# JacobYoung115/VisualSLAM

Hardware: AMD Instinct MI355X
Metric: frames/sec @1080p (Harris + DoG keypoint detection) (higher is better)
Workload: dtype u8

## Files before the change

### visualslam_amd/csrc/kernels_aux.hip.h

```cpp
#pragma once
#include <hip/hip_runtime.h>

#include "kernels_generic.hip.h"
#include "kernels_localize.hip.h"

namespace vslam {

__global__ __launch_bounds__(256) void k_resize_linear2x_slide(const uint8_t* __restrict__ src, size_t sstep, size_t sframe,
                                                                uint8_t* __restrict__ dst, size_t dframe, int dpitch,
                                                                int rows, int cols, int seg) {
    const int k = blockIdx.x * 256 + threadIdx.x;
    if (4 * k >= cols) return;
    const bool whole = 4 * k + 3 < cols;
    const int m0 = blockIdx.y * seg, m1 = min(m0 + seg, rows);
    const uint8_t* s = src + blockIdx.z * sframe;
    uint8_t* d = dst + blockIdx.z * dframe + 8 * k;
    const int xl = max(4 * k - 1, 0), xr = min(4 * k + 4, cols - 1);
    auto hrow = [&](int m, uint32_t (&X)[4], uint32_t (&Y)[4]) {
        const uint8_t* r = s + (size_t)min(max(m, 0), rows - 1) * sstep;
        uint32_t w;
        if (whole)
            __builtin_memcpy(&w, r + 4 * k, 4);
        else
            w = (uint32_t)r[4 * k] | ((uint32_t)r[min(4 * k + 1, cols - 1)] << 8) | ((uint32_t)r[min(4 * k + 2, cols - 1)] << 16) |
                ((uint32_t)r[cols - 1] << 24);
        const uint32_t s0 = r[xl], s5 = r[xr];
        const uint32_t P = __builtin_amdgcn_perm(w, w, 0x0c010c00);
        const uint32_t Q = __builtin_amdgcn_perm(w, w, 0x0c030c02);
        const uint32_t Qm = __builtin_amdgcn_perm(w, w, 0x0c020c01);
        const uint32_t Pm = s0 | ((w & 0xffu) << 16);
        const uint32_t Qp = (w >> 24) | (s5 << 16);
        const uint32_t P3 = P + (P << 1), Q3 = Q + (Q << 1);
        const uint32_t A[4] = {Pm + P3, P3 + Qm, Qm + Q3, Q3 + Qp};
#pragma unroll
        for (int i = 0; i < 4; ++i) {
            X[i] = pk_lshr_u16(A[i], 2);
            Y[i] = pk_lshr_u16(A[i] + (A[i] << 1), 2);
        }
    };
    auto emit = [&](int dy, const uint32_t (&U)[4], const uint32_t (&V)[4]) {
        uint32_t v[4];
#pragma unroll
        for (int i = 0; i < 4; ++i) v[i] = pk_lshr_u16(U[i] + V[i] + 0x00020002u, 2);
        *reinterpret_cast<uint2*>(d + (size_t)dy * dpitch) = make_uint2(v[0] | (v[1] << 8), v[2] | (v[3] << 8));
    };
    uint32_t Xp[4], Yp[4], Xc[4], Yc[4];
    hrow(m0 - 1, Xp, Yp);
    hrow(m0, Xc, Yc);
    for (int m = m0; m < m1; ++m) {
        uint32_t Xn[4], Yn[4];
        hrow(m + 1, Xn, Yn);
        emit(2 * m, Xp, Yc);
        emit(2 * m + 1, Yc, Xn);
#pragma unroll
        for (int i = 0; i < 4; ++i) Xp[i] = Xc[i], Xc[i] = Xn[i], Yc[i] = Yn[i];
    }
}

__global__ __launch_bounds__(256) void k_resize_nearest_half_v4(const uint8_t* __restrict__ src, size_t sframe, int spitch,
                                                                 uint8_t* __restrict__ dst, size_t dframe, int dpitch,
                                                                 int rows, int drows, int dcols) {
    const int k = blockIdx.x * 256 + threadIdx.x;
    const int y = blockIdx.y;
    if (4 * k >= dcols) return;
    const int sy = min(2 * y, rows - 1);
    const uint2 w = *reinterpret_cast<const uint2*>(src + blockIdx.z * sframe + (size_t)sy * spitch + 8 * k);
    *reinterpret_cast<uint32_t*>(dst + blockIdx.z * dframe + (size_t)y * dpitch + 4 * k) =
        even_bytes(w.x, w.y);
}

constexpr int EXT_SPAN = 768;
constexpr int EXT_PITCH = EXT_SPAN + 16;

template <bool LOC>
__global__ __launch_bounds__(256) void k_extrema_w3(const uint8_t* __restrict__ pyr, size_t pframe, ExtGeom g, int o,
                                                     unsigned long long* __restrict__ bits,
                                                     unsigned long long* __restrict__ lflags, size_t bframe, int li0, int li_step) {
    constexpr int NROW = LOC ? 13 : 10;
    __shared__ __attribute__((aligned(16))) uint8_t srow[NROW * EXT_PITCH + 16];
    __shared__ uint2 queue[LOC ? 768 : 1];
    __shared__ uint8_t qkeep[LOC ? 768 : 1];
    const int li = li0 + (int)blockIdx.y * li_step, f = blockIdx.z;
    const int rows = g.rows[o], cols = g.cols[o], pitch = g.pitch[o];
    const uint32_t P = (uint32_t)rows * (uint32_t)pitch;
    const uint8_t* dog = pyr + f * pframe + g.oct_off[o] + (size_t)VSLAM_NUM_LEVELS * P;
    const int ya = max(3 * li - 1, 0), yb = 3 * li;
    const int yc = min(3 * li + 1, rows - 1);
    const int c0 = blockIdx.x * EXT_SPAN - 16;
    const int wave = __builtin_amdgcn_readfirstlane(threadIdx.x >> 6), lane = threadIdx.x & 63;
    const int cpiece = c0 + 16 * lane;
    const bool piece_ok = lane < EXT_PITCH / 16 && cpiece >= 0 && cpiece < cols;
#pragma unroll
    for (int i = 0; i < (NROW + 3) / 4; ++i) {
        const int rl = wave + 4 * i;
        if (rl < NROW) {
            const int lev = rl < 10 ? (rl >> 1) : rl - 9, y = rl < 10 ? ((rl & 1) ? yb : ya) : yc;
            const uint8_t* rowp = dog + (ptrdiff_t)(int)((uint32_t)lev * P + (uint32_t)y * (uint32_t)pitch + (uint32_t)c0);
            if (piece_ok)
                *reinterpret_cast<uint4*>(srow + rl * EXT_PITCH + 16 * lane) =
                    *reinterpret_cast<const uint4*>(rowp + (uint32_t)(16 * lane));
        }
    }
    if (blockIdx.x == 0 && threadIdx.x < 10)
        srow[threadIdx.x * EXT_PITCH + 15] = dog[(threadIdx.x >> 1) * P + (uint32_t)((threadIdx.x & 1) ? yb : ya) * (uint32_t)pitch];
    __syncthreads();
    const int lc = g.lat_cols[o], wpr = g.wpr[o], lr = g.lat_rows[o];
    const int lj = blockIdx.x * 256 + threadIdx.x;
    bool cand[3] = {false, false, false}, listed[3] = {false, false, false};
    unsigned long long wcand[3], wlist[3];
    const unsigned long long owns = __builtin_amdgcn_ballot_w64(lj < lc);
    const int xa = 3 * (int)threadIdx.x - 1 + 16;
    uint32_t self[5];
    uint32_t up[5], left[5];
    {
        const uint32_t s = xa & 3;
        const uint32_t sel = 0x0c000c00u | s | ((s + 1) << 16);
        uint32_t mn[5], mx[5];
#pragma unroll
        for (int l = 0; l < 5; ++l) {
            uint32_t off = (uint32_t)(xa & ~3) + (uint32_t)(2 * l * EXT_PITCH);
            if (l) asm volatile("" : "+v"(off));
            const uint32_t* q0 = reinterpret_cast<const uint32_t*>(srow + off);
            const uint32_t* q1 = q0 + EXT_PITCH / 4;
            const uint32_t v0 = __builtin_amdgcn_perm(q0[1], q0[0], sel), v1 = __builtin_amdgcn_perm(q1[1], q1[0], sel);
            const uint32_t lo = pk_min_u16(v0, v1), hi = pk_max_u16(v0, v1);
            mn[l] = min(lo & 0xffffu, lo >> 16);
            mx[l] = max(hi & 0xffffu, hi >> 16);
            self[l] = v1 >> 16;
            if (LOC) up[l] = v0 >> 16, left[l] = v1 & 0xffffu;
        }
#pragma unroll
        for (int L = 1; L <= 3; ++L) {
            const uint32_t lo = min(mn[L - 1], min(mn[L], mn[L + 1])), hi = max(mx[L - 1], max(mx[L], mx[L + 1]));
            wcand[L - 1] = (__builtin_amdgcn_ballot_w64(self[L] == lo) | __builtin_amdgcn_ballot_w64(self[L] == hi)) & owns;
            if (LOC) cand[L - 1] = lj < lc && (self[L] == lo || self[L] == hi);
            else wlist[L - 1] = wcand[L - 1] & __builtin_amdgcn_ballot_w64((int)self[L] >= g.min_contrast);
        }
    }
    if (LOC) {
        uint2* wq = queue + wave * 192;
        uint8_t* wk = qkeep + wave * 192;
        const int xj = xa + 1;
        const int xr = xj + ((3 * lj + 1 < cols) ? 1 : 0);
        unsigned int nw = 0;
        bool queued[3];
#pragma unroll
        for (int L = 1; L <= 3; ++L) {
            bool nz = false;
            uint32_t dpack = 0;
            if (cand[L - 1]) {
                const uint8_t* r1 = srow + (2 * L + 1) * EXT_PITCH;
                const uint8_t* r2 = srow + (9 + L) * EXT_PITCH;
                const int d_x = (int)left[L] - (int)r1[xr];
                const int d_y = (int)up[L] - (int)r2[xj];
                const int d_s = (int)self[L - 1] - (int)self[L + 1];
                nz = d_x != 0 && d_y != 0 && d_s != 0;
                listed[L - 1] = !nz && self[L] >= 8u;
                dpack = (uint32_t)(d_x + 256) | ((uint32_t)(d_y + 256) << 10) | ((uint32_t)(d_s + 256) << 20);
            }
            const unsigned long long m = __builtin_amdgcn_ballot_w64(nz);
            if (nz) {
                const unsigned int slot = nw + __builtin_amdgcn_mbcnt_hi((uint32_t)(m >> 32), __builtin_amdgcn_mbcnt_lo((uint32_t)m, 0u));
                wq[slot] = make_uint2(dpack, self[L] | ((uint32_t)((L - 1) * 64 + lane) << 8));
            }
            queued[L - 1] = nz;
            nw += (unsigned int)__builtin_popcountll(m);
        }
        if (nw) {
            __builtin_amdgcn_fence(__ATOMIC_RELEASE, "wavefront");
            __builtin_amdgcn_wave_barrier();
            __builtin_amdgcn_fence(__ATOMIC_ACQUIRE, "wavefront");
            for (unsigned int q = lane; q < nw; q += 64) {
                const uint2 e = wq[q];
                int nv;
                wk[e.y >> 8] = feature_point_localization((int)(e.x & 1023u) - 256, (int)((e.x >> 10) & 1023u) - 256,
                                                          (int)(e.x >> 20) - 256, (int)(e.y & 255u), nv, g.loc_lut);
            }
            __builtin_amdgcn_fence(__ATOMIC_RELEASE, "wavefront");
            __builtin_amdgcn_wave_barrier();
            __builtin_amdgcn_fence(__ATOMIC_ACQUIRE, "wavefront");
#pragma unroll
            for (int L = 0; L < 3; ++L)
                if (queued[L]) listed[L] = wk[L * 64 + lane] != 0;
        }
    }
    const int word = blockIdx.x * 4 + wave;
    if (word < wpr) {
        const size_t w0 = f * bframe + g.bits_off[o] + (size_t)li * wpr + word;
#pragma unroll
        for (int L = 0; L < 3; ++L) {
            const unsigned long long wc = wcand[L], wl = LOC ? __builtin_amdgcn_ballot_w64(listed[L]) : wlist[L];
            if (lane == 0) {
                const size_t w = w0 + (size_t)L * lr * wpr;
                if (bits) bits[w] = wc;
                lflags[w] = wl;
            }
        }
    }
}


template <bool FMA>
__device__ __forceinline__ float mad_f32(float a, float b, float c) {
    if constexpr (FMA) return __builtin_fmaf(a, b, c);
    else return a * b + c;
}

template <bool FMA = false>
__device__ __forceinline__ float fast_atan2_deg(float y, float x) {
    const float scale = (float)(180.0 / 3.14159265358979323846);
    const float p1 = 0.9997878412794807f * scale, p3 = -0.3258083974640975f * scale;
    const float p5 = 0.1555786518463281f * scale, p7 = -0.04432655554792128f * scale;
    const float eps = (float)2.2204460492503131e-16;
    const float ax = fabsf(x), ay = fabsf(y);
    float a;
    if (ax >= ay) {
        const float c = ay / (ax + eps), c2 = c * c;
        a = mad_f32<FMA>(mad_f32<FMA>(mad_f32<FMA>(p7, c2, p5), c2, p3), c2, p1) * c;
    } else {
        const float c = ax / (ay + eps), c2 = c * c;
        a = 90.f - mad_f32<FMA>(mad_f32<FMA>(mad_f32<FMA>(p7, c2, p5), c2, p3), c2, p1) * c;
    }
    if (x < 0) a = 180.f - a;
    if (y < 0) a = 360.f - a;
    return a;
}

template <bool FMA>
__global__ __launch_bounds__(256) void k_level_gradients(const uint8_t* __restrict__ g, int gpitch, int rows, int cols,
                                                          float* __restrict__ gx, float* __restrict__ gy,
                                                          float* __restrict__ mag, float* __restrict__ orient) {
    const int c = blockIdx.x * 256 + threadIdx.x;
    const int r = blockIdx.y;
    if (c >= cols) return;
    float x, y;
    gradient_at(g, gpitch, rows, cols, r, c, x, y);
    const size_t o = (size_t)r * cols + c;
    if (gx) gx[o] = x;
    if (gy) gy[o] = y;
    if (mag) {
        const float xx = x * x, yy = y * y;
        mag[o] = sqrt_rn_small_nr(xx + yy);
    }
    if (orient) orient[o] = fast_atan2_deg<FMA>(y, x);
}

}
```

### visualslam_amd/csrc/vslam_hip.hip

```cpp
#include <hip/hip_runtime.h>

#include <algorithm>
#include <cstdio>
#include <cstdlib>
#include <cstring>
#include <deque>
#include <functional>
#include <map>
#include <string>
#include <set>
#include <memory>
#include <vector>

#include "../../include/vslam.h"
#include "kernels_generic.hip.h"
#include "kernels_pyramid.hip.h"
#include "kernels_strip.hip.h"
#include "kernels_hdiff.hip.h"
#include "kernels_aux.hip.h"
#include "kernels_harris_strip.hip.h"
#include "kernels_orient.hip.h"
#include "kernels_orient_batch.hip.h"
#include "kernels_orient_pk.hip.h"
#include "kernels_compact.hip.h"
#include "kernels_sift.hip.h"
#include "kernels_extrema_dense.hip.h"
#include "vslam_internal.h"
#include "vslam_ctx.h"
#include "vslam_launch.h"
#include "vslam_mx.h"
#include "vslam_octave_launch.h"

using namespace vslam;


struct vslam_pyramid {
    vslam_ctx* ctx = nullptr;
    vslam_params params{};
    vslam_batch_layout layout{};
    vslam_pyramid_info info{};
    uint8_t* d_block = nullptr;
    uint8_t* d_bases = nullptr;
    size_t block_cap = 0, bases_cap = 0;
    size_t base_off[VSLAM_MAX_OCTAVES] = {};
};


static const char* const kKernelNames =
    "k_resize_linear2x\nk_blur_h_generic\nk_blur_v_generic\n"
    "k_dog5\nk_resize_nearest_half\nk_extrema\nk_pyr_octave\nk_pyr_octave_mx\n"
    "k_gauss_v_strip\nk_gauss_h_strip\nk_gauss_h_diff\nk_resize_linear2x_slide\nk_resize_nearest_half_v4\nk_extrema_w3\nk_extrema_dense\nk_localize_points\nk_orient_keypoints\nk_edge_response_windows\nk_level_gradients\nk_pack_rows\nk_edge_flags\nk_survivor_ranges\nk_orient_survivors\n"
    "k_extrema_pack\nk_harris_strip\nk_flag_count\nk_chunk_scan\nk_flag_scatter\nk_level_gradients\nk_sift_descriptors\nk_pack_offsets\nk_pack_copy\nk_count_totals\n"
    "k_desc_norms\nk_match_nn2\nk_match_merge";


struct StreamSwap {
    vslam_ctx* c;
    hipStream_t saved;
    StreamSwap(vslam_ctx* ctx, hipStream_t s) : c(ctx), saved(ctx->stream) { c->stream = s; }
    ~StreamSwap() { c->stream = saved; }
};

static int raise_dyn_lds(vslam_ctx* c, const void* fn) {
    if (c->lds_raised.count(fn)) return VSLAM_OK;
    HIPCHK(c, hipFuncSetAttribute(fn, hipFuncAttributeMaxDynamicSharedMemorySize, kMaxDynLds));
    c->lds_raised.insert(fn);
    return VSLAM_OK;
}

static void* block_alloc(vslam_ctx* c, size_t bytes, size_t* cap) {
    int best = -1;
    for (int i = 0; i < (int)c->block_cache.size(); ++i) {
        const size_t sz = c->block_cache[i].first;
        if (sz >= bytes && sz <= 2 * bytes + (1 << 20) && (best < 0 || sz < c->block_cache[best].first)) best = i;
    }
    if (best >= 0) {
        void* p = c->block_cache[best].second;
        *cap = c->block_cache[best].first;
        c->block_cache.erase(c->block_cache.begin() + best);
        return p;
    }
    void* p = nullptr;
    if (hipMalloc(&p, bytes) != hipSuccess) {
        for (auto& b : c->block_cache) (void)hipFree(b.second);
        c->block_cache.clear();
        if (hipMalloc(&p, bytes) != hipSuccess) return nullptr;
    }
    *cap = bytes;
    return p;
}
static void block_release(vslam_ctx* c, void* p, size_t cap) {
    if (!p) return;
    if (c && c->block_cache.size() < 8 && cap <= ((size_t)1 << 30))
        c->block_cache.emplace_back(cap, p);
    else
        (void)hipFree(p);
}

int vslam::ws_reserve(vslam_ctx* c, size_t bytes) {
    if (bytes <= c->ws_cap) return VSLAM_OK;
    HIPCHK(c, hipStreamSynchronize(c->stream));
    for (int i = 0; i < vslam_ctx::kAux; ++i)
        if (c->aux[i]) HIPCHK(c, hipStreamSynchronize(c->aux[i]));
    if (c->ws) (void)hipFree(c->ws);
    c->ws = nullptr;
    c->ws_cap = 0;
    const size_t want = align_up(bytes + bytes / 8, 1 << 20);
    HIPCHK(c, hipMalloc((void**)&c->ws, want));
    c->ws_cap = want;
    return VSLAM_OK;
}

static bool stream_is_capturing(vslam_ctx* c) {
    hipStreamCaptureStatus cap = hipStreamCaptureStatusNone;
    if (hipStreamIsCapturing(c->stream, &cap) != hipSuccess) (void)hipGetLastError();
    return cap != hipStreamCaptureStatusNone;
}
#define NO_TABLE_IN_CAPTURE(ctx, what)                                                                                                      \
    if (stream_is_capturing(ctx))                                                                                                           \
    return fail(ctx, VSLAM_ERR_UNSUPPORTED, std::string(what) + ": its tap tables are not on the device yet and cannot be put there during a stream capture - " \
                                                                "run one warm-up call with the same parameters and the same matrix-path setting first")

enum TableKind { kTableBlur, kTableStrip, kTableTile, kTableMx, kTableOrient };

template <class T, class Fill>
static int get_table(vslam_ctx* c, TableKind kind, double v, int i, const char* what, size_t bytes, Fill fill, const T** out) {
    uint64_t vb;
    std::memcpy(&vb, &v, 8);
    const auto key = std::make_tuple((int)kind, vb, i);
    auto it = c->tables.find(key);
    if (it == c->tables.end()) {
        NO_TABLE_IN_CAPTURE(c, what);
        std::vector<char> host(bytes);
        TRY(fill(static_cast<void*>(host.data())));
// ... 262 lines not shown
    ws.add(s.bases, (size_t)nf * sum_p);
    ws.add(s.h, (size_t)nf * dog_h_elems(L, plans) + 128);
    ws.add(s.lflags, (size_t)nf * L.bits_frame_words);
    ws.add(s.cws, compaction_ws_elems(L.bits_frame_words, nf));
    ws.add(s.pbegin, nf);
}


template <class CFG>
static int enqueue_pyr_octave(vslam_ctx* c, double sigma0, int o, const OctPlan& pl, const OctIO& io) {
    const PyrTaps<CFG>* taps;
    TRY(get_table(c, kTableTile, sigma0, o, "octave kernel", sizeof(PyrTaps<CFG>), [&](void* host) -> int {
        const uint16_t* tp[6];
        tap_pointers(pl.taps, tp);
        pyr_pack_taps<CFG>(tp, *static_cast<PyrTaps<CFG>*>(host));
        return VSLAM_OK;
    }, &taps));
    TRY(raise_dyn_lds(c, reinterpret_cast<const void*>(&k_pyr_octave<CFG>)));
    const dim3 grid((io.cols + CFG::TW - 1) / CFG::TW, (io.rows + CFG::TH - 1) / CFG::TH, io.nf);
    LAUNCH_ON(c, "k_pyr_octave", o, c->stream, CFG::LDS_BYTES, k_pyr_octave<CFG>, grid, dim3(CFG::NT), io.base, io.bframe, io.oct, io.pframe, io.rows,
              io.cols, io.pitch, taps, io.next_base, io.nframe, io.nrows, io.ncols, io.npitch);
    return VSLAM_OK;
}

static int enqueue_pyr_octave_mx(vslam_ctx* c, double sigma0, int o, const OctPlan& pl, const OctIO& io, const MxScan* scan, int up2_step = 0) {
    const void* table;
    TRY(get_table(c, kTableMx, sigma0, o, "matrix-core octave kernel", mx_taps_bytes(pl.mx), [&](void* host) -> int {
        const uint16_t* tp[6];
        tap_pointers(pl.taps, tp);
        if (!mx_pack(pl.mx, tp, host)) return fail(c, VSLAM_ERR_UNSUPPORTED, "matrix-core octave kernel: a tap exceeds 127");
        HIPCHK(c, mx_prepare(pl.mx));
        return VSLAM_OK;
    }, &table));
    hipError_t e;
    {
        TimedScope ts(c, "k_pyr_octave_mx", o);
        e = mx_launch(pl.mx, c->stream, table, io, scan, up2_step);
    }
    HIPCHK(c, e);
    return VSLAM_OK;
}

static int dog_side_gate(const std::vector<OctPlan>& plans, int nf) {
    int gate = -1;
    if (nf >= 32)
        for (int o = 0; o < (int)plans.size(); ++o)
            if (plans[o].path == OctPath::Tile0 || plans[o].path == OctPath::Tile1) gate = o;
    return gate;
}

static DenseGeom dense_geom(const vslam_batch_layout& L, int o, int min_contrast, int nf) {
    DenseGeom g;
    g.rows = L.rows[o], g.cols = L.cols[o], g.pitch = L.pitch[o];
    g.wpr = (g.cols + 63) / 64;
    g.min_contrast = min_contrast;
    g.P = (unsigned int)((size_t)g.rows * g.pitch);
    g.dog_off = (unsigned int)(L.octave_offset[o] + (size_t)VSLAM_NUM_LEVELS * g.P);
    const long waves_per_rowseg = 4L * (((g.cols + 3) / 4 + 255) / 256) * nf;
    const long segs_wanted = std::max<long>(1, 8192 / waves_per_rowseg);
    g.seg = (int)std::min<long>(XD_SEG_MAX, std::max<long>(4, (g.rows + segs_wanted - 1) / segs_wanted));
    return g;
}

namespace {
struct DogOut {
    uint8_t* pyr;
    size_t pframe;
    unsigned long long* bits = nullptr;
    bool do_extrema = false;
    vslam_point* points = nullptr;
    unsigned int* counts = nullptr;
};

struct DogRun {
    hipStream_t side = nullptr;
    hipStream_t up = nullptr;
    std::function<int(int)> after_list;
    std::function<int(int)> after_octave;
    bool later_chunk = false;
    bool bases_are_scratch = false;
};
}

static int enqueue_octave_scan(vslam_ctx* c, const vslam_params& p, const vslam_batch_layout& L, const ExtGeom& g, const DogScratch& s,
                               const MxScan* fused, int o, int o_done, int nf, const DogOut& out, const DogRun& run) {
    uint8_t* const pyr = out.pyr;
    const size_t pframe = out.pframe;
    unsigned long long* const bits = out.bits;
    const hipStream_t side = run.side;
    if (out.do_extrema && L.lat_rows[o] > 0 && L.lat_cols[o] > 0) {
        hipStream_t es = c->stream;
        if (side) {
            HIPCHK(c, hipStreamWaitEvent(side, c->ev_oct[o_done], 0));
            es = side;
        }
        if (p.extrema_dense) {
            const DenseGeom dg = dense_geom(L, o, p.min_contrast, nf);
            hipLaunchKernelGGL(k_extrema_dense, dim3(((dg.cols + 3) / 4 + 255) / 256, (dg.rows + dg.seg - 1) / dg.seg, nf), dim3(256), 0, es,
                               pyr, pframe, dg, bits ? bits + L.bits_offset[o] : nullptr, s.lflags + L.bits_offset[o], L.bits_frame_words);
        } else if (fused) {
            {
                TimedScope ts(c, "k_extrema_pack", o, es);
                HIPCHK(c, mx_launch_pack(es, *fused, L.rows[o], L.lat_words[o], nf, bits ? bits + L.bits_offset[o] : nullptr, s.lflags + L.bits_offset[o],
                                         L.bits_frame_words, kMxStripRows));
            }
            const int sr = kMxStripRows;
            const int n_straddle = (L.lat_rows[o] - 1) / sr;
            TimedScope ts(c, "k_extrema_w3", o, es);
            if (n_straddle > 0)
                hipLaunchKernelGGL(k_extrema_w3<false>, dim3((L.lat_words[o] + 3) / 4, n_straddle, nf), dim3(256), 0, es, pyr, pframe, g, o, bits, s.lflags,
                                   L.bits_frame_words, sr, sr);
            if (es != c->stream) {
                HIPCHK(c, hipEventRecord(c->ev_pack, es));
                c->pack_pending = true;
            }
        } else if (p.extrema_window == 3) {
            const dim3 eg((L.lat_words[o] + 3) / 4, L.lat_rows[o], nf);
            if (p.localize)
                LAUNCH_ON(c, "k_extrema_w3", o, es, 0, k_extrema_w3<true>, eg, dim3(256), pyr, pframe, g, o, bits, s.lflags, L.bits_frame_words, 0, 1);
            else
                LAUNCH_ON(c, "k_extrema_w3", o, es, 0, k_extrema_w3<false>, eg, dim3(256), pyr, pframe, g, o, bits, s.lflags, L.bits_frame_words, 0, 1);
        } else
            hipLaunchKernelGGL(k_extrema, dim3((L.lat_cols[o] + 255) / 256, L.lat_rows[o], nf * 3), dim3(256), 0, es, pyr,
                               pframe, g, o, bits, s.lflags, L.bits_frame_words);
        HIPCHK(c, hipGetLastError());
    }
    if (out.do_extrema && out.points && out.counts) {
        StreamSwap sw(c, side ? side : c->stream);
        const size_t entries = (size_t)3 * L.lat_rows[o] * L.lat_words[o];
        if (p.extrema_dense) {
            DenseDogEntries ent{s.lflags + L.bits_offset[o], L.bits_frame_words, pyr, pframe, dense_geom(L, o, p.min_contrast, nf), o, out.points};
            TRY(enqueue_compaction(c, ent, entries, nf, s.cws, p.dog_cap, out.counts, o > 0 ? 1 : 0));
        } else {
            DogEntries ent{s.lflags, L.bits_frame_words, pyr, pframe, g, o, o + 1, out.points};
            TRY(enqueue_compaction(c, ent, entries, nf, s.cws, p.dog_cap, out.counts, o > 0 ? 1 : 0));
        }
        if (run.after_list) TRY(run.after_list(o));
    }
    return VSLAM_OK;
}

static int enqueue_dog(vslam_ctx* c, const vslam_params& p, const vslam_batch_layout& L, const std::vector<OctPlan>& plans, const uint8_t* frames,
                       size_t fstep, size_t fframe, int nf, DogScratch& s, const DogOut& out, const DogRun& run = DogRun()) {
    const hipStream_t side = run.side, up = run.up;
    const int gate = (side && p.localize) ? dog_side_gate(plans, nf) : -1;
    ExtGeom g;
    if (p.localize) TRY(ensure_loc_lut(c));
    fill_geom(c, p, L, g);
    const bool up2_fused = c->mx && run.bases_are_scratch && L.n_octaves > 0 && L.rows[0] == 2 * p.rows && L.cols[0] == 2 * p.cols && fstep <= 0x7fffffff &&
                           mx_up2_supported(plans[0].mx);
    const int nf_a = (!up2_fused && side && up && nf >= 64) ? nf / 2 : nf;
    if (!up2_fused)
        LAUNCH(c, "k_resize_linear2x_slide", k_resize_linear2x_slide, dim3(((p.cols + 3) / 4 + 255) / 256, (p.rows + 15) / 16, nf_a), dim3(256),
               frames, fstep, fframe, s.bases + s.base_off[0], s.bases_frame, L.pitch[0], p.rows, p.cols, 16);
    if (nf_a < nf) {
        if (run.later_chunk) HIPCHK(c, hipStreamWaitEvent(up, c->ev_chunk, 0));
        StreamSwap sw(c, up);
        LAUNCH(c, "k_resize_linear2x_slide", k_resize_linear2x_slide, dim3(((p.cols + 3) / 4 + 255) / 256, (p.rows + 15) / 16, nf - nf_a), dim3(256),
               frames + (size_t)nf_a * fframe, fstep, fframe, s.bases + s.base_off[0] + (size_t)nf_a * s.bases_frame, s.bases_frame, L.pitch[0],
               p.rows, p.cols, 16);
        HIPCHK(c, hipEventRecord(c->ev_up2, c->stream));
    }
    bool fused[VSLAM_MAX_OCTAVES] = {};
    if (run.later_chunk && c->pack_pending) {
        HIPCHK(c, hipStreamWaitEvent(c->stream, c->ev_pack, 0));
        c->pack_pending = false;
    }
    MxScan scan[VSLAM_MAX_OCTAVES] = {};
    struct TagReset {
        vslam_ctx* c;
        ~TagReset() { c->launch_tag = -1; }
    } tag_reset{c};
    for (int o = 0; o < L.n_octaves; ++o) {
        c->launch_tag = o;
        const int rows = L.rows[o], cols = L.cols[o], pitch = L.pitch[o];
        const size_t P = (size_t)rows * pitch;
        const OctPlan& pl = plans[o];
        const bool has_next = o + 1 < L.n_octaves;
        const bool fuse_next = has_next && pl.path != OctPath::Generic;
        OctIO io{s.bases + s.base_off[o], s.bases_frame, out.pyr + L.octave_offset[o], out.pframe, rows, cols, pitch, nf,
                 fuse_next ? s.bases + s.base_off[o + 1] : nullptr, s.bases_frame, has_next ? L.rows[o + 1] : 0, has_next ? L.cols[o + 1] : 0,
                 has_next ? L.pitch[o + 1] : 0};
        if (o == 0 && up2_fused) io.base = frames, io.bframe = fframe;
        const int shape = pyr_tile_wide(rows, cols) ? 1 : 0;
        fused[o] = c->mx && s.sitemap && out.do_extrema && !p.localize && !p.extrema_dense && p.extrema_window == 3 && L.lat_rows[o] > 0 &&
                   L.lat_cols[o] > 0 && mx_scan_supported(pl.mx);
        if (fused[o])
            scan[o] = MxScan{s.sitemap + s.site_off[o], s.site_frame, L.lat_rows[o], L.lat_cols[o], s.site_pitch[o], p.min_contrast,
                             s.colmap + s.col_off[o], s.col_frame, mx_seams(cols)};
        auto tiled = [&](int f_lo, int n) -> int {
            const OctIO part = io.frames(f_lo, n);
            if (c->mx && pl.mx) {
                MxScan sc = scan[o];
                if (fused[o]) sc.sitemap += (size_t)f_lo * s.site_frame, sc.colmap += (size_t)f_lo * s.col_frame;
                return enqueue_pyr_octave_mx(c, p.sigma0, o, pl, part, fused[o] ? &sc : nullptr, o == 0 && up2_fused ? (int)fstep : 0);
            }
            if (pl.path == OctPath::Tile0)
                return shape == 1 ? enqueue_pyr_octave<PyrCfgOct0W>(c, p.sigma0, o, pl, part) : enqueue_pyr_octave<PyrCfgOct0>(c, p.sigma0, o, pl, part);
            return shape == 1 ? enqueue_pyr_octave<PyrCfgOct1W>(c, p.sigma0, o, pl, part) : enqueue_pyr_octave<PyrCfgOct1>(c, p.sigma0, o, pl, part);
        };
        const bool is_tiled = pl.path == OctPath::Tile0 || pl.path == OctPath::Tile1 || (c->mx && pl.mx != 0);
        if (o == 0 && nf_a < nf && !is_tiled) HIPCHK(c, hipStreamWaitEvent(c->stream, c->ev_up2, 0));
        if (is_tiled && o == 0 && nf_a < nf) {
            TRY(tiled(0, nf_a));
// ... 461 lines not shown
    TRY(d2h(c, dst, dst_step, d_src, cols, cols, rows));
    return vslam_ctx_sync(c);
}

int vslam_pyramid_get_base(const vslam_pyramid* py, int octave, uint8_t* dst, size_t dst_step) {
    if (!py) return VSLAM_ERR_INVALID;
    if (octave < 0 || octave >= py->layout.n_octaves) return fail(py->ctx, VSLAM_ERR_RANGE, "octave out of range");
    return pyramid_fetch(py, octave, py->d_bases + py->base_off[octave], dst, dst_step);
}

int vslam_pyramid_get_gauss(const vslam_pyramid* py, int octave, int level, uint8_t* dst, size_t dst_step) {
    if (!py) return VSLAM_ERR_INVALID;
    if (octave < 0 || octave >= py->layout.n_octaves || level < 0 || level >= VSLAM_NUM_LEVELS)
        return fail(py->ctx, VSLAM_ERR_RANGE, "octave/level out of range");
    const size_t P = (size_t)py->layout.rows[octave] * py->layout.pitch[octave];
    return pyramid_fetch(py, octave, py->d_block + py->layout.octave_offset[octave] + (size_t)level * P, dst, dst_step);
}

int vslam_pyramid_get_dog(const vslam_pyramid* py, int octave, int level, uint8_t* dst, size_t dst_step) {
    if (!py) return VSLAM_ERR_INVALID;
    if (octave < 0 || octave >= py->layout.n_octaves || level < 0 || level >= VSLAM_NUM_DOGS)
        return fail(py->ctx, VSLAM_ERR_RANGE, "octave/level out of range");
    const size_t P = (size_t)py->layout.rows[octave] * py->layout.pitch[octave];
    return pyramid_fetch(py, octave,
                         py->d_block + py->layout.octave_offset[octave] + (size_t)(VSLAM_NUM_LEVELS + level) * P, dst,
                         dst_step);
}

int vslam_pyramid_get_gradients(const vslam_pyramid* py, int octave, int level, float* grad_x, float* grad_y, float* mag,
                                float* orient, size_t dst_step) {
    if (!py) return VSLAM_ERR_INVALID;
    vslam_ctx* c = py->ctx;
    TRY(bind_device(c));
    if (octave < 0 || octave >= py->layout.n_octaves || level < 0 || level >= VSLAM_NUM_LEVELS)
        return fail(c, VSLAM_ERR_RANGE, "octave/level out of range");
    const int rows = py->layout.rows[octave], cols = py->layout.cols[octave];
    ARGCHK(c, dst_step >= 4 * (size_t)cols, "pyramid gradients: bad destination step");
    float* host[4] = {grad_x, grad_y, mag, orient};
    const size_t P = (size_t)rows * cols;
    float* dev[4];
    WsPlan ws;
    for (int i = 0; i < 4; ++i) ws.add(dev[i], P);
    TRY(ws.commit(c));
    for (int i = 0; i < 4; ++i)
        if (!host[i]) dev[i] = nullptr;
    const int pitch = py->layout.pitch[octave];
    const uint8_t* g = py->d_block + py->layout.octave_offset[octave] + (size_t)level * rows * pitch;
    if (c->f32_fused)
        LAUNCH(c, "k_level_gradients", k_level_gradients<true>, grid_rows(cols, rows), dim3(256), g, pitch, rows, cols, dev[0], dev[1], dev[2], dev[3]);
    else
        LAUNCH(c, "k_level_gradients", k_level_gradients<false>, grid_rows(cols, rows), dim3(256), g, pitch, rows, cols, dev[0], dev[1], dev[2], dev[3]);
    for (int i = 0; i < 4; ++i)
        if (host[i]) TRY(d2h(c, host[i], dst_step, dev[i], 4 * (size_t)cols, 4 * (size_t)cols, rows));
    return vslam_ctx_sync(c);
}

static int dog_points_host(vslam_ctx* c, const vslam_pyramid* py, int octave, int window, int min_contrast, int localize,
                           uint64_t* bits, vslam_point* out, size_t cap, size_t* count) {
    TRY(bind_device(c));
    ARGCHK(c, py && py->ctx == c && count && (out || cap == 0), "initialKeypointDetection: bad arguments");
    if (octave < 0 || octave >= py->layout.n_octaves) return fail(c, VSLAM_ERR_RANGE, "octave out of range");
    ARGCHK(c, window >= 3 && (window & 1), "initialKeypointDetection: windowSize must be odd and >= 3");
    vslam_params p = py->params;
    p.extrema_window = window;
    p.min_contrast = min_contrast;
    p.localize = localize;
    p.dog_cap = (uint32_t)std::min<size_t>(cap, 0x7fffffff);
    vslam_batch_layout L;
    if (make_layout(&p, &L) != VSLAM_OK) return fail(c, VSLAM_ERR_INVALID, "bad extrema parameters");
    ExtGeom g;
    if (p.localize) TRY(ensure_loc_lut(c));
    fill_geom(c, p, L, g);
    const size_t words = L.bits_frame_words;
    unsigned long long *d_bits, *d_lf;
    vslam_point* d_pts;
    unsigned int *d_n, *d_cws;
    WsPlan ws;
    ws.add(d_bits, words), ws.add(d_lf, words), ws.add(d_pts, p.dog_cap), ws.add(d_n, 1), ws.add(d_cws, compaction_ws_elems(words, 1));
    TRY(ws.commit(c));
    HIPCHK(c, hipMemsetAsync(d_n, 0, 4, c->stream));
    const size_t ow = (size_t)3 * L.lat_rows[octave] * L.lat_words[octave];
    if (ow) {
        if (window == 3) {
            const dim3 eg((L.lat_words[octave] + 3) / 4, L.lat_rows[octave], 1);
            if (localize)
                LAUNCH(c, "k_extrema_w3", k_extrema_w3<true>, eg, dim3(256), py->d_block, L.pyramid_frame_bytes, g, octave, d_bits, d_lf, words, 0, 1);
            else
                LAUNCH(c, "k_extrema_w3", k_extrema_w3<false>, eg, dim3(256), py->d_block, L.pyramid_frame_bytes, g, octave, d_bits, d_lf, words, 0, 1);
        } else {
            LAUNCH(c, "k_extrema", k_extrema, dim3((L.lat_cols[octave] + 255) / 256, L.lat_rows[octave], 3), dim3(256),
                   py->d_block, L.pyramid_frame_bytes, g, octave, d_bits, d_lf, words);
        }
        DogEntries ent{d_lf, words, py->d_block, L.pyramid_frame_bytes, g, octave, octave + 1, d_pts};
        TRY(enqueue_compaction(c, ent, ow, 1, d_cws, p.dog_cap, d_n, 0));
    }
    return read_list(c, d_n, d_pts, p.dog_cap, out, count, bits, d_bits + L.bits_offset[octave], bits ? ow * 8 : 0);
}

int vslam_dog_extrema(vslam_ctx* c, const vslam_pyramid* py, int octave, int window, int min_contrast, uint64_t* bits,
                      vslam_point* out, size_t cap, size_t* count) {
    return dog_points_host(c, py, octave, window, min_contrast, 0, bits, out, cap, count);
}

int vslam_dog_extrema_dense(vslam_ctx* c, const vslam_pyramid* py, int octave, int min_contrast, uint64_t* bits,
                            vslam_point* out, size_t cap, size_t* count) {
    TRY(bind_device(c));
    ARGCHK(c, py && py->ctx == c && count && (out || cap == 0), "dense extrema: bad arguments");
    if (octave < 0 || octave >= py->layout.n_octaves) return fail(c, VSLAM_ERR_RANGE, "octave out of range");
    ARGCHK(c, min_contrast >= 0 && min_contrast <= 65535, "dense extrema: min_contrast out of range");
    const vslam_batch_layout& L = py->layout;
    DenseGeom g = dense_geom(L, octave, min_contrast, 1);
    const size_t words = (size_t)3 * g.rows * g.wpr;
    const unsigned int ocap = (unsigned int)std::min<size_t>(cap, 0x7fffffff);
    unsigned long long *d_bits, *d_lf;
    vslam_point* d_pts;
    unsigned int *d_n, *d_cws;
    WsPlan ws;
    ws.add(d_bits, words), ws.add(d_lf, words), ws.add(d_pts, ocap), ws.add(d_n, 1), ws.add(d_cws, compaction_ws_elems(words, 1));
    TRY(ws.commit(c));
    HIPCHK(c, hipMemsetAsync(d_n, 0, 4, c->stream));
    LAUNCH(c, "k_extrema_dense", k_extrema_dense, dim3(((g.cols + 3) / 4 + 255) / 256, (g.rows + g.seg - 1) / g.seg, 1), dim3(256),
           py->d_block, L.pyramid_frame_bytes, g, bits ? d_bits : nullptr, d_lf, words);
    DenseDogEntries ent{d_lf, words, py->d_block, L.pyramid_frame_bytes, g, octave, d_pts};
    TRY(enqueue_compaction(c, ent, words, 1, d_cws, ocap, d_n, 0));
    return read_list(c, d_n, d_pts, ocap, out, count, bits, d_bits, bits ? words * 8 : 0);
}

int vslam_dog_keypoints(vslam_ctx* c, const vslam_pyramid* py, int octave, int window, vslam_point* out, size_t cap,
                        size_t* count) {
    return dog_points_host(c, py, octave, window, 0, 1, nullptr, out, cap, count);
}

int vslam_localize_points(vslam_ctx* c, const int* diffs, size_t n, int* keep, int* value) {
    TRY(bind_device(c));
    ARGCHK(c, (diffs && keep && value) || n == 0, "FeaturePointLocalization: bad arguments");
    ARGCHK(c, n <= 0x7fffffff, "FeaturePointLocalization: too many points");
    if (n == 0) return VSLAM_OK;
    int4* d_in;
    int2* d_out;
    WsPlan ws;
    ws.add(d_in, n), ws.add(d_out, n);
    TRY(ws.commit(c));
    HIPCHK(c, hipMemcpyAsync(d_in, diffs, 16 * n, hipMemcpyHostToDevice, c->stream));
    TRY(ensure_loc_lut(c));
    LAUNCH(c, "k_localize_points", k_localize_points, dim3((unsigned)((n + 255) / 256)), dim3(256), d_in, (int)n, d_out, c->loc_lut);
    std::vector<int2> h(n);
    HIPCHK(c, hipMemcpyAsync(h.data(), d_out, 8 * n, hipMemcpyDeviceToHost, c->stream));
    TRY(vslam_ctx_sync(c));
    for (size_t i = 0; i < n; ++i) keep[i] = h[i].x, value[i] = h[i].y;
    return VSLAM_OK;
}

int vslam_filter_keypoints(vslam_ctx* c, const vslam_pyramid* py, int octave, const vslam_point* kps, size_t n,
                           vslam_point* out, size_t cap, size_t* count) {
    TRY(bind_device(c));
    ARGCHK(c, py && py->ctx == c && count && (kps || n == 0) && (out || cap == 0), "filterKeypoints: bad arguments");
    if (octave < 0 || octave >= py->layout.n_octaves) return fail(c, VSLAM_ERR_RANGE, "octave out of range");
    ARGCHK(c, n <= 0x7fffffff, "filterKeypoints: too many keypoints");
    *count = 0;
    if (n == 0) return VSLAM_OK;
    const int rows = py->layout.rows[octave], cols = py->layout.cols[octave], pitch = py->layout.pitch[octave];
    const size_t P = (size_t)rows * cols;
    bool used[VSLAM_NUM_LEVELS] = {};
    for (size_t i = 0; i < n; ++i) {
        const vslam_point& k = kps[i];
        if (k.level < 0 || k.level >= VSLAM_NUM_LEVELS || k.col < 0 || k.row < 0 || k.col > cols || k.row > rows || k.octave != octave)
            return fail(c, VSLAM_ERR_RANGE, "filterKeypoints: keypoint outside the octave's data");
        used[k.level] = true;
    }
    std::vector<float> taps[VSLAM_NUM_LEVELS];
    int max_r = 0;
// ... 577 lines not shown
```

### visualslam_amd/csrc/vslam_octave_launch.h

```cpp
#pragma once
#include <algorithm>
#include <cstddef>
#include <initializer_list>

namespace vslam {

constexpr int STRIP_W = 64;
constexpr int HD_J = 16;
constexpr int HD_PAD = 2;
constexpr int kMaxDynLds = 150 * 1024;

struct StripVGeom {
    int RM, rhq;
    size_t lds;
};
constexpr StripVGeom strip_v_geom(int rows, int nmax) {
    const int RM = (nmax / 2 + 3) & ~3;
    const int rhq = (((rows + 3) & ~3) + 2 * RM + 16) / 4;
    return StripVGeom{RM, rhq, (size_t)rhq * STRIP_W * 4};
}

constexpr int strip_pw(int cols, int nmax) { return ((cols + 7) / 2 + nmax / 2 + 12 + 3) & ~3; }

constexpr int strip_item_capacity(int RI) { return RI == 4 ? 512 : 1024; }

constexpr int strip_sh(int cols) { return cols <= 1024 ? 16 : cols <= 2048 ? 8 : cols <= 4096 ? 4 : 0; }

constexpr int strip_plan_sh(int rows, int cols, int nmax) {
    const int sh = strip_sh(cols);
    return sh && strip_v_geom(rows, nmax).lds <= (size_t)kMaxDynLds && (size_t)sh * strip_pw(cols, nmax) * 4 <= (size_t)kMaxDynLds ? sh : 0;
}

constexpr int hd_left_halo(int rmax) { return (rmax + 2 + 15) & ~15; }
constexpr int hd_pw(int cols, int HL, int rmax) {
    const int ccount = HL + 16 * ((cols + HD_J - 1) / HD_J) + rmax;
    return (ccount + 1 + 15) / 16 * (16 + HD_PAD);
}
constexpr bool hdiff_fits(int cols) { return (cols + HD_J - 1) / HD_J <= 256; }

struct StripLaunch {
    int lsplit;
    size_t v_lds;
    bool diff;
    int npairs;
    int SH, RI;
    int h_grid_y;
    size_t h_lds;
    int pw;
};

inline StripLaunch strip_launch(int rows, int cols, int nf, int sh, bool hdiff, int nmax, int hd_HL = 0, int hd_rmax = 0) {
    StripLaunch s{};
    s.v_lds = strip_v_geom(rows, nmax).lds;
    const int strips = (cols + STRIP_W - 1) / STRIP_W;
    const int want = (256 + strips * nf - 1) / (strips * nf);
    s.lsplit = want >= 6 ? 6 : want >= 3 ? 3 : want >= 2 ? 2 : 1;
    if (hdiff) {
        const int ncs = (cols + HD_J - 1) / HD_J;
        s.pw = hd_pw(cols, hd_HL, hd_rmax);
        int npairs = std::max(1, std::min(8, 256 / ncs));
        while (npairs > 1 && ((size_t)npairs * s.pw * 8 > (size_t)kMaxDynLds || (long)((rows + 2 * npairs - 1) / (2 * npairs)) * nf < 256)) --npairs;
        s.diff = true;
        s.npairs = npairs;
        s.h_grid_y = (rows + 2 * npairs - 1) / (2 * npairs);
        s.h_lds = (size_t)npairs * s.pw * 8;
        return s;
    }
    s.pw = strip_pw(cols, nmax);
    while (sh > 4 && (long)((rows + sh - 1) / sh) * nf < 256) sh >>= 1;
    int ri = 4;
    if (sh == 4 && (long)((rows + 3) / 4) * nf < 256 && ((cols + 7) / 8) * 4 <= 512) {
        ri = 1;
    } else if (sh == 16) {
        const int ncg = (cols + 7) / 8;
        auto waste = [&](int r) {
            const long items = (long)ncg * (16 / r);
            if (items > strip_item_capacity(r)) return 1e9;
            return (double)((items + 63) / 64 * 64 - items) / (double)items;
        };
        for (int r : {2, 1})
            if (waste(r) + 0.02 < waste(ri)) ri = r;
    }
    s.SH = sh;
    s.RI = ri;
    s.h_grid_y = (rows + sh - 1) / sh;
    s.h_lds = (size_t)sh * s.pw * 4;
    return s;
}

constexpr bool pyr_tile_wide(int rows, int cols) {
    return (long)((cols + 255) / 256) * ((rows + 31) / 32) <= (long)((cols + 127) / 128) * ((rows + 63) / 64);
}

}
```

Baseline: 14580.

## Add paired-row 3x3x3 extrema scan kernel processing two lattice rows per block

Adds k_extrema_w3_pairs, a 128-thread kernel that stages four DoG rows per level into LDS and evaluates two lattice rows per block. It uses byte-perm packing and packed 16-bit min/max to test both rows at once, sharing the overlapping middle rows. A launch helper picks this path for full, non-localized scans and otherwise falls back to the existing kernel. The aim is fewer redundant row loads and less per-row launch overhead, at the cost of smaller blocks and extra bookkeeping for the edge guard and odd row counts.

```diff
diff --git a/visualslam_amd/csrc/kernels_aux.hip.h b/visualslam_amd/csrc/kernels_aux.hip.h
--- a/visualslam_amd/csrc/kernels_aux.hip.h
+++ b/visualslam_amd/csrc/kernels_aux.hip.h
@@ -3,6 +3,7 @@
 
 #include "kernels_generic.hip.h"
 #include "kernels_localize.hip.h"
+#include "vslam_octave_launch.h"
 
 namespace vslam {
 
@@ -69,8 +70,6 @@
         even_bytes(w.x, w.y);
 }
 
-constexpr int EXT_SPAN = 768;
-constexpr int EXT_PITCH = EXT_SPAN + 16;
 
 template <bool LOC>
 __global__ __launch_bounds__(256) void k_extrema_w3(const uint8_t* __restrict__ pyr, size_t pframe, ExtGeom g, int o,
@@ -199,6 +198,90 @@
     }
 }
 
+typedef __attribute__((address_space(3))) uint32_t lds_u32;
+struct __attribute__((aligned(8))) ExtPiece {
+    uint2 lo, hi;
+};
+
+__global__ __launch_bounds__(EXT2_SITES) void k_extrema_w3_pairs(const uint8_t* __restrict__ pyr, size_t pframe, ExtGeom g, int o,
+                                                                  unsigned long long* __restrict__ bits,
+                                                                  unsigned long long* __restrict__ lflags, size_t bframe) {
+    __shared__ __attribute__((aligned(16))) uint8_t srow[EXT2_ROWS * EXT2_PITCH];
+    const int li = 2 * (int)blockIdx.y, f = blockIdx.z;
+    const int rows = g.rows[o], cols = g.cols[o], pitch = g.pitch[o];
+    const uint32_t P = (uint32_t)rows * (uint32_t)pitch;
+    const int wave = __builtin_amdgcn_readfirstlane(threadIdx.x >> 6), lane = threadIdx.x & 63;
+    const int c0 = (int)blockIdx.x * EXT2_SPAN - EXT2_GUARD;
+    {
+        const int y0 = wave ? min(3 * li + 2, rows - 1) : max(3 * li - 1, 0), y1 = wave ? min(3 * li + 3, rows - 1) : 3 * li;
+        const uint8_t* lev = pyr + f * pframe + g.oct_off[o] + (size_t)VSLAM_NUM_LEVELS * P + (ptrdiff_t)c0;
+        const uint32_t o0 = (uint32_t)y0 * (uint32_t)pitch, o1 = (uint32_t)y1 * (uint32_t)pitch;
+        const int at = min(min(16 * lane, EXT2_PITCH - 16), pitch - 16 - c0);
+        const bool piece_ok = 16 * lane < EXT2_PITCH && c0 + 16 * lane < cols;
+        uint8_t* dst = srow + (2 * wave) * EXT2_PITCH + at;
+#pragma unroll
+        for (int l = 0; l < 5; ++l) {
+            if (piece_ok) {
+                ExtPiece a = *reinterpret_cast<const ExtPiece*>(lev + o0 + (uint32_t)at);
+                ExtPiece b = *reinterpret_cast<const ExtPiece*>(lev + o1 + (uint32_t)at);
+                *reinterpret_cast<ExtPiece*>(dst + (4 * l) * EXT2_PITCH) = a;
+                *reinterpret_cast<ExtPiece*>(dst + (4 * l + 1) * EXT2_PITCH) = b;
+            }
+            lev += P;
+        }
+    }
+    __syncthreads();
+    if (blockIdx.x == 0) {
+        if (threadIdx.x < EXT2_ROWS) srow[threadIdx.x * EXT2_PITCH + EXT2_GUARD - 1] = srow[threadIdx.x * EXT2_PITCH + EXT2_GUARD];
+        __syncthreads();
+    }
+    const int lc = g.lat_cols[o], wpr = g.wpr[o], lr = g.lat_rows[o];
+    const int lj = (int)blockIdx.x * EXT2_SITES + (int)threadIdx.x;
+    const unsigned long long owns = __builtin_amdgcn_ballot_w64(lj < lc);
+    const uint32_t xa = 3u * threadIdx.x + (EXT2_GUARD - 1), xb = xa + 1;
+    const uint32_t sela = 0x0c040c00u + (xa & 3) * 0x00010001u, selb = 0x0c040c00u + (xb & 3) * 0x00010001u;
+    const uint8_t* pa = srow + (xa & ~3u);
+    const uint8_t* pb = srow + (xb & ~3u);
+    uint32_t mn[5], mx[5], self[5];
+#pragma unroll
+    for (int l = 0; l < 5; ++l) {
+        uint32_t a[4], b[4];
+#pragma unroll
+        for (int r = 0; r < 4; ++r) {
+            a[r] = *(const volatile lds_u32*)(pa + (4 * l + r) * EXT2_PITCH);
+            b[r] = *(const volatile lds_u32*)(pb + (4 * l + r) * EXT2_PITCH);
+        }
+        const uint32_t a02 = __builtin_amdgcn_perm(a[2], a[0], sela), b02 = __builtin_amdgcn_perm(b[2], b[0], selb);
+        const uint32_t a13 = __builtin_amdgcn_perm(a[3], a[1], sela), b13 = __builtin_amdgcn_perm(b[3], b[1], selb);
+        mn[l] = pk_min_u16(pk_min_u16(a02, b02), pk_min_u16(a13, b13));
+        mx[l] = pk_max_u16(pk_max_u16(a02, b02), pk_max_u16(a13, b13));
+        self[l] = b13;
+    }
+    unsigned long long wc[3][2], wl[3][2];
+#pragma unroll
+    for (int L = 1; L <= 3; ++L) {
+        const uint32_t lo = pk_min_u16(mn[L - 1], pk_min_u16(mn[L], mn[L + 1])), hi = pk_max_u16(mx[L - 1], pk_max_u16(mx[L], mx[L + 1]));
+        const uint32_t s0 = self[L] & 0xffffu, s1 = self[L] >> 16;
+        wc[L - 1][0] = (__builtin_amdgcn_ballot_w64(s0 == (lo & 0xffffu)) | __builtin_amdgcn_ballot_w64(s0 == (hi & 0xffffu))) & owns;
+        wc[L - 1][1] = (__builtin_amdgcn_ballot_w64(s1 == (lo >> 16)) | __builtin_amdgcn_ballot_w64(s1 == (hi >> 16))) & owns;
+        wl[L - 1][0] = wc[L - 1][0] & __builtin_amdgcn_ballot_w64((int)s0 >= g.min_contrast);
+        wl[L - 1][1] = wc[L - 1][1] & __builtin_amdgcn_ballot_w64((int)s1 >= g.min_contrast);
+    }
+    const int word = (int)blockIdx.x * 2 + wave;
+    if (word < wpr && lane == 0) {
+        const int nrow = li + 1 < lr ? 2 : 1;
+        const size_t w0 = f * bframe + g.bits_off[o] + (size_t)((uint32_t)li * (uint32_t)wpr + (uint32_t)word);
+        const size_t lstep = (uint32_t)lr * (uint32_t)wpr;
+        for (int r = 0; r < nrow; ++r) {
+            unsigned long long* lf = lflags + w0 + (uint32_t)(r * wpr);
+            lf[0] = r ? wl[0][1] : wl[0][0], lf[lstep] = r ? wl[1][1] : wl[1][0], lf[2 * lstep] = r ? wl[2][1] : wl[2][0];
+            if (bits) {
+                unsigned long long* bt = bits + w0 + (uint32_t)(r * wpr);
+                bt[0] = r ? wc[0][1] : wc[0][0], bt[lstep] = r ? wc[1][1] : wc[1][0], bt[2 * lstep] = r ? wc[2][1] : wc[2][0];
+            }
+        }
+    }
+}
 
 template <bool FMA>
 __device__ __forceinline__ float mad_f32(float a, float b, float c) {
diff --git a/visualslam_amd/csrc/vslam_hip.hip b/visualslam_amd/csrc/vslam_hip.hip
--- a/visualslam_amd/csrc/vslam_hip.hip
+++ b/visualslam_amd/csrc/vslam_hip.hip
@@ -49,7 +49,7 @@
 static const char* const kKernelNames =
     "k_resize_linear2x\nk_blur_h_generic\nk_blur_v_generic\n"
     "k_dog5\nk_resize_nearest_half\nk_extrema\nk_pyr_octave\nk_pyr_octave_mx\n"
-    "k_gauss_v_strip\nk_gauss_h_strip\nk_gauss_h_diff\nk_resize_linear2x_slide\nk_resize_nearest_half_v4\nk_extrema_w3\nk_extrema_dense\nk_localize_points\nk_orient_keypoints\nk_edge_response_windows\nk_level_gradients\nk_pack_rows\nk_edge_flags\nk_survivor_ranges\nk_orient_survivors\n"
+    "k_gauss_v_strip\nk_gauss_h_strip\nk_gauss_h_diff\nk_resize_linear2x_slide\nk_resize_nearest_half_v4\nk_extrema_w3\nk_extrema_w3_pairs\nk_extrema_dense\nk_localize_points\nk_orient_keypoints\nk_edge_response_windows\nk_level_gradients\nk_pack_rows\nk_edge_flags\nk_survivor_ranges\nk_orient_survivors\n"
     "k_extrema_pack\nk_harris_strip\nk_flag_count\nk_chunk_scan\nk_flag_scatter\nk_level_gradients\nk_sift_descriptors\nk_pack_offsets\nk_pack_copy\nk_count_totals\n"
     "k_desc_norms\nk_match_nn2\nk_match_merge";
 
@@ -478,6 +478,26 @@
 };
 }
 
+#ifdef VSLAM_DIAGNOSTICS
+static bool g_scan_pairs = true;
+extern "C" __attribute__((visibility("default"))) void vslam_diag_scan_pairs(int on) { g_scan_pairs = on != 0; }
+#else
+static constexpr bool g_scan_pairs = true;
+#endif
+
+static int launch_scan_w3(vslam_ctx* c, hipStream_t st, const uint8_t* pyr, size_t pframe, const ExtGeom& g, int o, bool localize, int li0, int li_step,
+                          int n_rows, int nf, unsigned long long* bits, unsigned long long* lflags, size_t bframe) {
+    const ScanLaunch sl = scan_launch(g.lat_rows[o], g.lat_cols[o], localize, li0, li_step, n_rows, g_scan_pairs);
+    const dim3 grid(sl.grid_x, sl.grid_y, nf), block(sl.threads);
+    if (sl.pairs)
+        LAUNCH_ON(c, "k_extrema_w3", o, st, 0, k_extrema_w3_pairs, grid, block, pyr, pframe, g, o, bits, lflags, bframe);
+    else if (localize)
+        LAUNCH_ON(c, "k_extrema_w3", o, st, 0, k_extrema_w3<true>, grid, block, pyr, pframe, g, o, bits, lflags, bframe, li0, li_step);
+    else
+        LAUNCH_ON(c, "k_extrema_w3", o, st, 0, k_extrema_w3<false>, grid, block, pyr, pframe, g, o, bits, lflags, bframe, li0, li_step);
+    return VSLAM_OK;
+}
+
 static int enqueue_octave_scan(vslam_ctx* c, const vslam_params& p, const vslam_batch_layout& L, const ExtGeom& g, const DogScratch& s,
                                const MxScan* fused, int o, int o_done, int nf, const DogOut& out, const DogRun& run) {
     uint8_t* const pyr = out.pyr;
@@ -502,20 +522,16 @@
             }
             const int sr = kMxStripRows;
             const int n_straddle = (L.lat_rows[o] - 1) / sr;
-            TimedScope ts(c, "k_extrema_w3", o, es);
             if (n_straddle > 0)
-                hipLaunchKernelGGL(k_extrema_w3<false>, dim3((L.lat_words[o] + 3) / 4, n_straddle, nf), dim3(256), 0, es, pyr, pframe, g, o, bits, s.lflags,
-                                   L.bits_frame_words, sr, sr);
+                TRY(launch_scan_w3(c, es, pyr, pframe, g, o, false, sr, sr, n_straddle, nf, bits, s.lflags, L.bits_frame_words));
+            else
+                TimedScope ts(c, "k_extrema_w3", o, es);
             if (es != c->stream) {
                 HIPCHK(c, hipEventRecord(c->ev_pack, es));
                 c->pack_pending = true;
             }
         } else if (p.extrema_window == 3) {
-            const dim3 eg((L.lat_words[o] + 3) / 4, L.lat_rows[o], nf);
-            if (p.localize)
-                LAUNCH_ON(c, "k_extrema_w3", o, es, 0, k_extrema_w3<true>, eg, dim3(256), pyr, pframe, g, o, bits, s.lflags, L.bits_frame_words, 0, 1);
-            else
-                LAUNCH_ON(c, "k_extrema_w3", o, es, 0, k_extrema_w3<false>, eg, dim3(256), pyr, pframe, g, o, bits, s.lflags, L.bits_frame_words, 0, 1);
+            TRY(launch_scan_w3(c, es, pyr, pframe, g, o, p.localize != 0, 0, 1, L.lat_rows[o], nf, bits, s.lflags, L.bits_frame_words));
         } else
             hipLaunchKernelGGL(k_extrema, dim3((L.lat_cols[o] + 255) / 256, L.lat_rows[o], nf * 3), dim3(256), 0, es, pyr,
                                pframe, g, o, bits, s.lflags, L.bits_frame_words);
@@ -1143,11 +1159,7 @@
     const size_t ow = (size_t)3 * L.lat_rows[octave] * L.lat_words[octave];
     if (ow) {
         if (window == 3) {
-            const dim3 eg((L.lat_words[octave] + 3) / 4, L.lat_rows[octave], 1);
-            if (localize)
-                LAUNCH(c, "k_extrema_w3", k_extrema_w3<true>, eg, dim3(256), py->d_block, L.pyramid_frame_bytes, g, octave, d_bits, d_lf, words, 0, 1);
-            else
-                LAUNCH(c, "k_extrema_w3", k_extrema_w3<false>, eg, dim3(256), py->d_block, L.pyramid_frame_bytes, g, octave, d_bits, d_lf, words, 0, 1);
+            TRY(launch_scan_w3(c, c->stream, py->d_block, L.pyramid_frame_bytes, g, octave, localize != 0, 0, 1, L.lat_rows[octave], 1, d_bits, d_lf, words));
         } else {
             LAUNCH(c, "k_extrema", k_extrema, dim3((L.lat_cols[octave] + 255) / 256, L.lat_rows[octave], 3), dim3(256),
                    py->d_block, L.pyramid_frame_bytes, g, octave, d_bits, d_lf, words);
diff --git a/visualslam_amd/csrc/vslam_octave_launch.h b/visualslam_amd/csrc/vslam_octave_launch.h
--- a/visualslam_amd/csrc/vslam_octave_launch.h
+++ b/visualslam_amd/csrc/vslam_octave_launch.h
@@ -88,6 +88,31 @@
     return s;
 }
 
+constexpr int EXT_SPAN = 768;
+constexpr int EXT_PITCH = EXT_SPAN + 16;
+constexpr size_t ext_lds(bool localize) { return (size_t)(localize ? 13 : 10) * EXT_PITCH + 16 + (localize ? 768 * 8 + 768 : 0); }
+constexpr int EXT2_SITES = 128;
+constexpr int EXT2_SPAN = 3 * EXT2_SITES;
+constexpr int EXT2_GUARD = 8;
+constexpr int EXT2_PITCH = EXT2_SPAN + EXT2_GUARD;
+constexpr int EXT2_ROWS = 20;
+constexpr size_t ext2_lds() { return (size_t)EXT2_ROWS * EXT2_PITCH; }
+static_assert(ext2_lds() <= ext_lds(false), "the pair scan must fit where the plain scan does");
+
+struct ScanLaunch {
+    bool pairs;
+    int threads;
+    int grid_x, grid_y;
+    size_t lds;
+};
+
+inline ScanLaunch scan_launch(int lat_rows, int lat_cols, bool localize, int li0, int li_step, int n_rows, bool pairs_on = true) {
+    const int words = (lat_cols + 63) / 64;
+    if (pairs_on && !localize && li0 == 0 && li_step == 1 && n_rows == lat_rows)
+        return ScanLaunch{true, EXT2_SITES, (lat_cols + EXT2_SITES - 1) / EXT2_SITES, (lat_rows + 1) / 2, ext2_lds()};
+    return ScanLaunch{false, 256, (words + 3) / 4, n_rows, ext_lds(localize)};
+}
+
 constexpr bool pyr_tile_wide(int rows, int cols) {
     return (long)((cols + 255) / 256) * ((rows + 31) / 32) <= (long)((cols + 127) / 128) * ((rows + 63) / 64);
 }
```

Measured after the change: 14040. 0.963x the previous value.
